# rlorenzo/facet

Measured on AMD Instinct MI355X. Metric: images/sec whole-node (TOPIQ+SAMP+CLIP+InsightFace ensemble), 1024² batch, higher is better.
Workload: dtype f32

## Files before the change

### facet_amd/_lib.py

```python
import ctypes as C
import importlib.util
import os
import sys
import threading

import numpy as np

_HERE = os.path.dirname(os.path.abspath(__file__))
LIB_PATH = os.environ.get("FACET_AMD_LIB") or os.path.join(_HERE, "libfacet_engine.so")

FE_MODEL_TOPIQ, FE_MODEL_CLIP, FE_MODEL_SAMP, FE_MODEL_U2NETP, FE_MODEL_AESTHETIC, FE_MODEL_VLM = range(6)
FE_RECORD_FLOATS = 789
FE_GRAPH_FACE_DET, FE_GRAPH_FACE_LMK, FE_GRAPH_FACE_REC = 0, 1, 2
FE_FACE_FLOATS = 739
FE_STATS_DOUBLES = 264
FILTERS = {"lanczos": 1, "bilinear": 2, "bicubic": 3}
FE_PRECISION_RES32 = 16
FE_PRECISION_SPLIT3 = 32
PRECISION = {"f32": 0, "fp32": 0, "float32": 0, "bf16": 1, "bfloat16": 1, "f16": 2, "fp16": 2, "float16": 2, "half": 2,
             "bf16+r32": 1 | FE_PRECISION_RES32, "f16+r32": 2 | FE_PRECISION_RES32, "f16x3": 2 | FE_PRECISION_RES32 | FE_PRECISION_SPLIT3}
PRECISION_NAME = {0: "f32", 1: "bf16", 2: "f16", 1 | FE_PRECISION_RES32: "bf16+r32", 2 | FE_PRECISION_RES32: "f16+r32",
                  2 | FE_PRECISION_RES32 | FE_PRECISION_SPLIT3: "f16x3"}
ACT = {"none": 0, None: 0, "relu": 1, "gelu": 2, "sigmoid": 3, "softplus": 5, "quickgelu": 6}
ELEM = {"f32": 0, "bf16": 1, "f16": 2}
# ... 31 lines not shown
SIGNATURES = {
    "fe_create": (C.c_int, [C.c_int, C.c_size_t, C.POINTER(C.c_void_p)]),
    "fe_destroy": (None, [C.c_void_p]),
    "fe_last_error": (C.c_char_p, [C.c_void_p]),
    "fe_version": (C.c_char_p, []),
    "fe_sync": (C.c_int, [C.c_void_p]),
    "fe_set_microbatch": (C.c_int, [C.c_void_p, C.c_int]),
    "fe_set_precision": (C.c_int, [C.c_void_p, C.c_int]),
    "fe_model_precision": (C.c_int, [C.c_void_p, C.c_int]),
    "fe_dev_alloc": (C.c_int, [C.c_void_p, C.c_size_t, C.POINTER(C.c_void_p)]),
    "fe_dev_free": (C.c_int, [C.c_void_p, C.c_void_p]),
    "fe_memcpy_h2d": (C.c_int, [C.c_void_p, C.c_void_p, C.c_void_p, C.c_size_t]),
    "fe_memcpy_d2h": (C.c_int, [C.c_void_p, C.c_void_p, C.c_void_p, C.c_size_t]),
    "fe_timer_start": (C.c_int, [C.c_void_p]),
    "fe_timer_stop": (C.c_int, [C.c_void_p, _f32p]),
    "fe_profile_enable": (C.c_int, [C.c_void_p, C.c_int]),
    "fe_profile_count": (C.c_int, [C.c_void_p]),
    "fe_profile_get": (C.c_int, [C.c_void_p, C.c_int, C.c_char_p, C.c_int, C.POINTER(C.c_double),
                                 C.POINTER(C.c_double), _f32p]),
    "fe_flops_reset": (C.c_int, [C.c_void_p]),
    "fe_flops_get": (C.c_int, [C.c_void_p, C.POINTER(C.c_double)]),
    "fe_flops_get_executed": (C.c_int, [C.c_void_p, C.POINTER(C.c_double)]),
    "fe_flops_get_half": (C.c_int, [C.c_void_p, C.POINTER(C.c_double)]),
    "fe_weights_begin": (C.c_int, [C.c_void_p, C.c_int]),
    "fe_weights_set": (C.c_int, [C.c_void_p, C.c_int, C.c_char_p, _f32p, _i64p, C.c_int]),
    "fe_weights_commit": (C.c_int, [C.c_void_p, C.c_int]),
    "fe_model_unload": (C.c_int, [C.c_void_p, C.c_int]),
    "fe_model_loaded": (C.c_int, [C.c_void_p, C.c_int]),
    "fe_op_conv2d": (C.c_int, [C.c_void_p, _f32p, C.c_int, C.c_int, C.c_int, C.c_int, _f32p, C.c_int, C.c_int,
                               C.c_int, _f32p, _f32p, _f32p, C.c_int, C.c_int, C.c_int, C.c_int, C.c_int, _f32p]),
    "fe_op_gate_rowpool": (C.c_int, [C.c_void_p, _f32p, C.c_int, C.c_int, C.c_int, C.c_int, C.c_int, _f32p, _f32p, C.c_int, _f32p, C.c_int,
                                     C.c_int, C.c_int, C.c_int, _f32p, C.POINTER(C.c_int)]),
    "fe_op_wino64": (C.c_int, [C.c_void_p, _f32p, C.c_int, C.c_int, C.c_int, C.c_int, _f32p, C.c_int, _f32p, _f32p, _f32p, C.c_int, C.c_int, _f32p]),
    "fe_op_topiq_gate64": (C.c_int, [C.c_void_p, _f32p, C.c_int, C.c_int, C.c_int, _f32p, _f32p, _f32p, _f32p, _f32p, C.c_float,
                                     _f32p, _f32p, C.c_int, C.c_int, _f32p]),
    "fe_op_conv3x3_c64": (C.c_int, [C.c_void_p, _f32p, C.c_int, C.c_int, C.c_int, _f32p, _f32p, _f32p, C.c_int, _f32p, _f32p, _f32p,
                                    _f32p, _f32p]),
    "fe_op_maxpool2d": (C.c_int, [C.c_void_p, _f32p, C.c_int, C.c_int, C.c_int, C.c_int, C.c_int, C.c_int,
                                  C.c_int, C.c_int, _f32p]),
    "fe_op_bilinear": (C.c_int, [C.c_void_p, _f32p, C.c_int, C.c_int, C.c_int, C.c_int, C.c_int, C.c_int, _f32p]),
    "fe_op_adaptive_avgpool": (C.c_int, [C.c_void_p, _f32p, C.c_int, C.c_int, C.c_int, C.c_int, C.c_int, C.c_int,
                                         _f32p]),
    "fe_op_layernorm": (C.c_int, [C.c_void_p, _f32p, C.c_int, C.c_int, _f32p, _f32p, C.c_float, _f32p]),
    "fe_op_plane": (C.c_int, [C.c_void_p, C.c_int, C.c_int, _f32p] + [C.c_int] * 14 + [C.c_float, C.c_float, _f32p]),
    "fe_op_rowpass": (C.c_int, [C.c_void_p, C.c_int, C.c_int, C.c_int, _f32p] + [C.c_int] * 6 + [_f32p, _f32p, C.c_int, C.c_int, C.c_float, C.c_float, _f32p]),
    "fe_op_gemm_skinny": (C.c_int, [C.c_void_p, C.c_int, C.c_int, C.c_int, _f32p, C.c_int, C.c_int, C.c_int, _f32p, C.c_int, C.c_int, _f32p, _f32p, C.c_int,
                                    C.c_int, C.c_float, _f32p]),
    "fe_op_gemm_skinny_res": (C.c_int, [C.c_void_p, C.c_int, C.c_int, C.c_int, _f32p, C.c_int, C.c_int, C.c_int, _f32p, C.c_int, C.c_int, _f32p, _f32p, _f32p,
                                        C.c_int, C.c_int, C.c_int, C.c_float, _f32p]),
    "fe_op_attention": (C.c_int, [C.c_void_p, _f32p, _f32p, _f32p, _f32p, C.c_int, C.c_int, C.c_int, C.c_int, C.c_int, C.c_int, _f32p]),
    "fe_op_mha": (C.c_int, [C.c_void_p, _f32p, _f32p, C.c_int, C.c_int, C.c_int, C.c_int, C.c_int, _f32p, _f32p, _f32p, _f32p, _f32p,
                            C.c_int, _f32p]),
    "fe_op_vlm_select": (C.c_int, [C.c_void_p, _f32p, C.c_int, C.c_int, C.POINTER(C.c_int32), _f32p]),
    "fe_op_vlm_decode_attention": (C.c_int, [C.c_void_p, _f32p, _f32p, _f32p, C.c_int, C.c_int, C.c_int, C.c_int, C.POINTER(C.c_int32), C.c_int, C.c_int,
                                             _f32p, _f32p, _f32p]),
    "fe_op_vlm_linear": (C.c_int, [C.c_void_p, _f32p, C.c_int, C.c_int, _f32p, _f32p, C.c_int, C.c_int, C.c_int, _f32p, _f32p, _f32p, C.c_float,
                                   C.POINTER(C.c_int32), _f32p, C.c_int, C.c_int, C.c_int, _f32p, _f32p, C.POINTER(C.c_int32)]),
    "fe_op_vlm_rope_cache": (C.c_int, [C.c_void_p, _f32p, C.POINTER(C.c_int32), _f32p, C.c_int, _f32p, _f32p, C.c_float] + [C.c_int] * 12 +
                             [_f32p, C.POINTER(C.c_uint8), C.POINTER(C.c_uint8), _f32p, _f32p]),
    "fe_op_vlm_rows": (C.c_int, [C.c_void_p, C.c_int, _f32p, _f32p, _f32p, C.POINTER(C.c_int32), _f32p, C.c_int, C.c_int, C.c_int, C.c_int, C.c_int,
                                 C.c_float, C.c_int, C.c_int, _f32p, _f32p]),
    "fe_op_vlm_vis_rope": (C.c_int, [C.c_void_p, _f32p, C.POINTER(C.c_int32), _f32p, C.c_int, C.c_int, C.c_int, C.c_int, _f32p, _f32p]),
    "fe_op_vlm_vis_attention": (C.c_int, [C.c_void_p, _f32p, _f32p, _f32p, C.POINTER(C.c_int32), C.c_int, C.c_int, C.c_int, C.c_int, _f32p]),
    "fe_op_vlm_prefill_attention": (C.c_int, [C.c_void_p, _f32p, _f32p, _f32p] + [C.c_int] * 6 + [C.POINTER(C.c_int32), _f32p]),
    "fe_set_conv_variant": (C.c_int, [C.c_void_p, C.c_int]),
    "fe_bench_conv": (C.c_int, [C.c_void_p] + [C.c_int] * 12 + [_f32p]),
# ... 396 lines not shown
        xr, xp = _f32(xr)
        weight, wp = _f32(weight)
        cout = weight.shape[0]
        assert weight.shape == (cout, cin)
        bp = None
        if bias is not None:
            bias, bp = _f32(bias)
        gate, gp = _f32(gate)
        assert gate.shape == (n, h, w)
        y = np.empty((n, th, tw, cout), np.float32)
        routed = C.c_int(0)
        self._ck(self.lib.fe_op_gate_rowpool(self.h, xp, n, h, w, cin, ldx, wp, bp, cout, gp, ACT[act], th, tw, int(bool(fused)),
                                             y.ctypes.data_as(_f32p), C.byref(routed)))
        return np.ascontiguousarray(y.transpose(0, 3, 1, 2)), bool(routed.value)

    def wino64_conv(self, x, w, scale=None, shift=None, res=None, res_after_act=False, act=None):
        x, xp = _f32(x)
        w, wp = _f32(w)
        n, c, h, ww = x.shape
        cout = w.shape[0]
        assert w.shape == (cout, c, 3, 3)
        y = np.empty((n, cout, h, ww), np.float32)
        sp = hp = rp = None
        if scale is not None:
            scale, sp = _f32(scale)
        if shift is not None:
            shift, hp = _f32(shift)
        if res is not None:
            res, rp = _f32(res)
            assert res.shape == y.shape
        self._ck(self.lib.fe_op_wino64(self.h, xp, n, c, h, ww, wp, cout, sp, hp, rp, int(res_after_act), ACT[act], y.ctypes.data_as(_f32p)))
        return y

    def topiq_gate64(self, x, w0, b0, w2, b2, w4, b4, wx, bx, wblk_act="gelu", gate_act="gelu"):
        x, xp = _f32(x)
        n, c, h, w = x.shape
        assert c == 64
        arrs = [_f32(a) for a in (w0, b0, w2, b2, w4, wx, bx)]
        y = np.empty((n, 64, h // 16, w // 16), np.float32)
        self._ck(self.lib.fe_op_topiq_gate64(self.h, xp, n, h, w, arrs[0][1], arrs[1][1], arrs[2][1], arrs[3][1], arrs[4][1], C.c_float(float(b4)),
                                             arrs[5][1], arrs[6][1], ACT[wblk_act], ACT[gate_act], y.ctypes.data_as(_f32p)))
        return y

    def conv3x3_c64(self, x, w2, scale2=None, shift2=None, act2="relu", w3=None, scale3=None, shift3=None, res=None):
        x, xp = _f32(x)
        n, c, h, w = x.shape
        assert c == 64
        keep = [_f32(a) if a is not None else (None, None) for a in (w2, scale2, shift2, w3, scale3, shift3, res)]
        y = np.empty((n, 256 if w3 is not None else 64, h, w), np.float32)
        self._ck(self.lib.fe_op_conv3x3_c64(self.h, xp, n, h, w, keep[0][1], keep[1][1], keep[2][1], ACT[act2], keep[3][1], keep[4][1], keep[5][1],
                                            keep[6][1], y.ctypes.data_as(_f32p)))
        return y

    def maxpool2d(self, x, k, stride, pad=0, ceil_mode=False):
        x, xp = _f32(x)
        n, c, h, w = x.shape

        def od(i):
            if ceil_mode:
                o = -(-(i + 2 * pad - k) // stride) + 1
                if (o - 1) * stride >= i + pad:
                    o -= 1
                return o
            return (i + 2 * pad - k) // stride + 1
        y = np.empty((n, c, od(h), od(w)), np.float32)
        self._ck(self.lib.fe_op_maxpool2d(self.h, xp, n, c, h, w, k, stride, pad, int(ceil_mode),
# ... 1315 lines not shown
```

### facet_amd/csrc/capi_ops.hip

```cpp
#include "capi_internal.h"
#include "fp8_core.h"
#include "wino64_maps.h"

template <class E>
static E* hook_up(Ctx& C, const float* src, size_t n, int off = 0) {
  if (!src) return nullptr;
  if constexpr (std::is_same_v<E, float>) {
    float* d = C.arena.array<float>(n + off) + off;
    FE_HIP(hipMemcpyAsync(d, src, n * sizeof(float), hipMemcpyHostToDevice, C.stream));
    return d;
  } else {
    const float* d32 = upload(C, src, n);
    E* d = C.arena.array<E>(n + off) + off;
    launch_convert(d32, d, n, C.stream);
    return d;
  }
}
template <class E>
static E* hook_filled(Ctx& C, size_t n, float fill, int off = 0) {
  const std::vector<float> v(n, fill);
  E* d = hook_up<E>(C, v.data(), n, off);
  FE_HIP(hipStreamSynchronize(C.stream));
  return d;
}
// ... 123 lines not shown
    FE_HIP(hipMemcpyAsync(xt.p, x, xt.numel() * sizeof(float), hipMemcpyHostToDevice, C.stream));
    Tensor gt = C.arena.tensor(n, h, w, 1);
    FE_HIP(hipMemcpyAsync(gt.p, gate, gt.numel() * sizeof(float), hipMemcpyHostToDevice, C.stream));
    ConvOpts og; og.act = act; og.gate = &gt;
    int took = 0;
    Tensor pooled = topiq_gate_pool(C, cw, xt.slice(0, cw.CinPad), og, th, tw, fused != 0, &took);
    FE_CHECK(pooled.h == th && pooled.w == tw && pooled.ld == cout, "fe_op_gate_rowpool: unexpected result shape");
    FE_HIP(hipMemcpyAsync(y, pooled.p, pooled.numel() * sizeof(float), hipMemcpyDeviceToHost, C.stream));
    FE_HIP(hipStreamSynchronize(C.stream));
    if (routed) *routed = took;
  });
}

int fe_op_wino64(fe_ctx* ctx, const float* x, int n, int c, int h, int w, const float* weight, int cout, const float* scale, const float* shift,
                 const float* res, int res_after_act, int act, float* y) {
  return fe_api(ctx, [&] {
    Ctx& C = ctx->c;
    FE_CHECK(x && weight && y && n > 0 && h > 0 && w > 0 && c > 0 && c <= 64 && c % 4 == 0 && cout > 0 && cout <= 64 && cout % 4 == 0, "bad wino64 arguments");
    FE_CHECK(C.precision == PREC_F32, "fe_op_wino64: fp32 contexts only");
    C.arena.reset();
    std::vector<float> U(w64::U_FLOATS);
    w64::pack_u(weight, cout, c, U.data());
    const float* dU = upload(C, U.data(), U.size());
    const float *ds = upload(C, scale, (size_t)cout), *dh = upload(C, shift, (size_t)cout);
    Tensor xt = upload_nchw(C, x, n, c, h, w, c);
    Tensor rt;
    if (res) rt = upload_nchw(C, res, n, cout, h, w, cout);
    Tensor yt = C.arena.tensor(n, h, w, cout);
    launch_wino64(xt, yt, dU, ds, dh, nullptr, act, res ? &rt : nullptr, res_after_act, C.stream);
    download_nchw(C, yt, cout, y);
  });
}

int fe_op_topiq_gate64(fe_ctx* ctx, const float* x, int n, int h, int w, const float* w0, const float* b0, const float* w2, const float* b2,
                       const float* w4, float b4, const float* wx, const float* bx, int wblk_act, int gate_act, float* y) {
  return fe_api(ctx, [&] {
    Ctx& C = ctx->c;
    FE_CHECK(x && w0 && b0 && w2 && b2 && w4 && wx && bx && y && n > 0 && h > 0 && w > 0 && h % 16 == 0 && w % 16 == 0, "bad gate64 arguments");
    FE_CHECK(C.precision == PREC_BF16 || C.precision == PREC_F16, "fe_op_topiq_gate64: the fused gate exists for the 2-byte element types only");
    C.arena.reset();
    DeviceWeights dw;
    dw.prec = C.precision;
    GatedConvW g;
    build_gate64_fragments(dw, g, w0, b0, w2, b2, w4, b4, wx, bx);
    auto run = [&](auto* tag) {
      typedef std::remove_pointer_t<decltype(tag)> E;
      TensorT<E> xt = upload_nchw<E>(C, x, n, 64, h, w, 64);
      TensorT<E> yt = C.arena.tensor_t<E>(n, h / 16, w / 16, 64);
      launch_topiq_gate64(xt, yt, g.fused, g.fused_bias, wblk_act, gate_act, C.stream);
      download_nchw(C, yt, 64, y);
    };
    if (C.precision == PREC_BF16) run((bf16*)nullptr); else run((f16*)nullptr);
  });
}

int fe_op_conv3x3_c64(fe_ctx* ctx, const float* x, int n, int h, int w, const float* w2, const float* scale2, const float* shift2, int act2,
                      const float* w3, const float* scale3, const float* shift3, const float* res, float* y) {
  return fe_api(ctx, [&] {
    Ctx& C = ctx->c;
    FE_CHECK(x && w2 && y && n > 0 && h > 0 && w > 0 && (!w3 || res), "bad conv3x3_c64 arguments");
    FE_CHECK(C.precision == PREC_BF16 || C.precision == PREC_F16, "fe_op_conv3x3_c64: the halo-tiled kernel exists for the 2-byte element types only");
    C.arena.reset();
    DeviceWeights dw;
    dw.prec = C.precision;
    void *f2 = nullptr, *f3 = nullptr;
    build_c64_fragments(dw, w2, w3, &f2, &f3);
// ... 618 lines not shown
```

### facet_amd/csrc/engine.hip

```cpp
#include "engine.h"
#include "onnx_graph.h"
#include "wino64_maps.h"
#include <algorithm>
#include <cmath>
#include <cstdlib>

namespace fe {

void WeightStore::set(const std::string& name, const float* data, const int64_t* shape, int ndim) {
  HostTensor h;
  h.shape.assign(shape, shape + ndim);
  h.data.assign(data, data + h.numel());
  t_[name] = std::move(h);
}
const HostTensor& WeightStore::get(const std::string& name) const {
  auto it = t_.find(name);
  if (it == t_.end()) throw Error("missing weight tensor '" + name + "'");
  return it->second;
}

float* DeviceWeights::upload(const std::vector<float>& v) {
  void* p = nullptr;
  const size_t b = v.size() * sizeof(float);
  FE_HIP(hipMalloc(&p, b ? b : 16));
// ... 225 lines not shown
}

bool conv_wino64(Ctx& c, const ConvW& w, const Tensor& x, const Tensor& y, const ConvOpts& o) {
  if (!(w.wino64 && c.force_variant == 0 && w.KH == 3 && w.KW == 3 && o.sh == 1 && o.sw == 1 && o.ph == 1 && o.pw == 1 && o.dh == 1 && o.dw == 1 && !o.gate && !o.pool_kw &&
        x.c == w.CinPad && y.c == w.Cout && y.n == x.n && y.h == x.h && y.w == x.w &&
        (((uintptr_t)x.p | (uintptr_t)y.p | (uintptr_t)(o.res ? o.res->p : nullptr)) & 15) == 0 && x.ld % 4 == 0 && y.ld % 4 == 0 &&
        (!o.res || o.res->ld % 4 == 0) && (unsigned long long)x.h * x.w * x.ld * 4ull < 0xF0000000ull && y.pixels() < (1ull << 31)))
    return false;
  const int M = (int)y.pixels();
  hipEvent_t e0 = nullptr, e1 = nullptr;
  if (c.profile) {
    FE_HIP(hipEventCreate(&e0)); FE_HIP(hipEventCreate(&e1));
    FE_HIP(hipEventRecord(e0, c.stream));
  }
  launch_wino64(x, y, w.wino64, w.scale, w.shift, w.slope, o.act, o.res, o.res_after_act, c.stream);
  const double direct = 2.0 * M * (double)(9 * w.Cin) * (w.CoutAlg ? w.CoutAlg : w.Cout);
  if (c.profile) {
    FE_HIP(hipEventRecord(e1, c.stream));
    FE_HIP(hipEventSynchronize(e1));
    float ms = 0.f;
    FE_HIP(hipEventElapsedTime(&ms, e0, e1));
    (void)hipEventDestroy(e0); (void)hipEventDestroy(e1);
    char nm[128];
    snprintf(nm, sizeof nm, "wino64 3x3 M=%d K=%d N=%d", M, w.K, w.Cout);
    const double bytes = 4.0 * ((double)x.pixels() * x.c + (double)y.pixels() * y.c * (o.res ? 2 : 1) + (double)w64::U_FLOATS);
    c.timings.push_back({nm, direct, bytes, ms});
  }
  const double tiles = (double)x.n * ((x.h + 1) / 2) * ((x.w + 1) / 2);
  c.flops_accum += direct;
  c.flops_saved += direct - 2.0 * 16.0 * tiles * 64.0 * w.Cout;
  return true;
}

void conv_forward(Ctx& c, const ConvW& w, const Tensor& x, const Tensor& y, const ConvOpts& o) {
  FE_CHECK(x.c == w.CinPad, "conv: input channels %d != packed Cin %d", x.c, w.CinPad);
  FE_CHECK(y.c == w.Cout && y.n == x.n, "conv: output view mismatch (c=%d Cout=%d)", y.c, w.Cout);
  ConvParams p{};
  p.x = x.p; p.ldx = x.ld;
  p.w = w.w; p.scale = w.scale; p.shift = w.shift; p.slope = w.slope;
  FE_CHECK(o.act != ACT_PRELU || w.slope, "conv: PReLU without slopes");
  if (o.res) {
    FE_CHECK(o.res->c == y.c && o.res->pixels() == y.pixels(), "conv: residual shape mismatch");
    p.res = o.res->p; p.ldr = o.res->ld;
  }
  if (o.gate) {
    FE_CHECK(o.gate->pixels() == y.pixels() && (o.gate->c == 1 || o.gate->c == y.c), "conv: gate shape mismatch");
    p.gate = o.gate->p; p.ldg = o.gate->ld; p.gate_c1 = o.gate->c == 1;
  }
  p.y = y.p; p.ldy = y.ld;
  p.N = x.n; p.H = x.h; p.W = x.w; p.Cin = w.CinPad;
  p.Ho = y.h; p.Wo = y.w; p.Cout = w.Cout;
  p.KH = w.KH; p.KW = w.KW; p.sh = o.sh; p.sw = o.sw; p.ph = o.ph; p.pw = o.pw; p.dh = o.dh; p.dw = o.dw;
  FE_CHECK(y.h == conv_out_dim(x.h, w.KH, o.sh, o.ph, o.dh) && y.w == conv_out_dim(x.w, w.KW, o.sw, o.pw, o.dw),
           "conv: output dims %dx%d inconsistent with input %dx%d", y.h, y.w, x.h, x.w);
  p.K = w.K; p.Kp = w.Kp;
  p.M = (int)y.pixels();
  FE_CHECK(y.pixels() < (1ull << 31), "conv: M too large");
  p.act = o.act; p.res_after_act = o.res_after_act;
  p.variant = c.force_variant;
  if (o.pool_kw) {
    FE_CHECK(conv_rowpool_ok(c, w, x, o, o.pool_kw), "conv: the row-pooling epilogue does not apply to this layer (kw=%d)", o.pool_kw);
    FE_CHECK(o.pool && o.pool->p && o.pool->n == x.n && o.pool->h == x.h && o.pool->w * o.pool_kw == x.w && o.pool->c == w.Cout, "conv: pool view mismatch");
    p.pool_kw = o.pool_kw; p.pool = o.pool->p; p.ldp = o.pool->ld;
    p.y = nullptr; p.ldy = w.Cout;
  }
  if (w.wtap && o.act != ACT_PRELU && o.sh == 1 && o.sw == 1 && !o.res && !o.gate && p.variant == 0 && y.h == x.h && y.w == x.w) {
    const int T = w.KH * w.KW * w.Cout, Tp = (T + 3) & ~3;
    const size_t mark = c.arena.mark();
    Tensor z = c.arena.tensor(x.n, x.h, x.w, Tp);
    ConvParams q{};
    q.x = x.p; q.ldx = x.ld; q.w = w.wtap; q.y = z.p; q.ldy = Tp;
    q.N = x.n; q.H = x.h; q.W = x.w; q.Cin = w.CinPad; q.Ho = x.h; q.Wo = x.w; q.Cout = T;
    q.KH = q.KW = 1; q.sh = q.sw = q.dh = q.dw = 1;
    q.K = w.CinPad; q.Kp = w.KpT; q.M = (int)x.pixels();
    launch_conv(q, c.stream);
    launch_tap_gather(z.p, Tp, x.n, x.h, x.w, w.KH, w.KW, o.ph, o.pw, o.dh, o.dw, w.Cout, w.scale, w.shift, o.act, y.p,
                      y.ld, y.h, y.w, c.stream);
    c.arena.rewind(mark);
    c.flops_accum += 2.0 * p.M * (double)(w.KH * w.KW * w.Cin) * (w.CoutAlg ? w.CoutAlg : p.Cout);
    return;
  }
  static const bool no_wino = getenv("FE_NO_WINO") != nullptr;
  const bool wino_plain = !o.res && (o.act == ACT_NONE || o.act == ACT_RELU);
  if (w.wino && !no_wino && p.variant == 0 && o.sh == 1 && o.sw == 1 && o.ph == 1 && o.pw == 1 && o.dh == 1 && o.dw == 1 &&
      !o.gate && (wino_plain || (w.wino_m == 4 && (o.act == ACT_NONE || o.act == ACT_RELU || o.act == ACT_PRELU))) && y.h == x.h && y.w == x.w && (((uintptr_t)x.p | (uintptr_t)y.p) & 15) == 0 &&
      x.ld % 4 == 0 && y.ld % 4 == 0) {
    const int ts = w.wino_m, planes = (ts + 2) * (ts + 2);
    const int th = (x.h + ts - 1) / ts, tw = (x.w + ts - 1) / ts;
    const size_t tiles = (size_t)x.n * th * tw;
    const size_t wino_bytes = (size_t)planes * tiles * ((size_t)w.CinPad + w.Cout) * sizeof(float) + 1024;
    if (tiles < (1u << 30) / 36 && c.arena.mark() + wino_bytes <= c.arena.capacity()) {
      const size_t mark = c.arena.mark();
      float* V = (float*)c.arena.alloc((size_t)planes * tiles * w.CinPad * sizeof(float));
      float* Mb = (float*)c.arena.alloc((size_t)planes * tiles * w.Cout * sizeof(float));
      hipEvent_t e0 = nullptr, e1 = nullptr;
      if (c.profile) {
        FE_HIP(hipEventCreate(&e0)); FE_HIP(hipEventCreate(&e1));
        FE_HIP(hipEventRecord(e0, c.stream));
      }
      if (ts == 2) launch_wino_input(x, th, tw, V, c.stream);
      else launch_wino4_input(x, th, tw, V, c.stream);
      ConvParams g{};
      g.x = V; g.ldx = w.CinPad; g.w = w.wino; g.ldw = w.CinPad; g.y = Mb; g.ldy = w.Cout;
      g.M = (int)tiles; g.K = w.CinPad; g.Cout = w.Cout;
      g.N = 1; g.H = 1; g.W = g.M; g.Ho = 1; g.Wo = g.M; g.KH = g.KW = 1; g.sh = g.sw = g.dh = g.dw = 1;
      g.Kp = w.CinPad; g.Cin = w.CinPad;
      g.batch = planes; g.nb1 = 1; g.xs2 = (long long)tiles * w.CinPad; g.ws2 = (long long)w.Cout * w.CinPad; g.ys2 = (long long)tiles * w.Cout;
      launch_conv(g, c.stream);
      if (ts == 2) launch_wino_output(Mb, y, th, tw, w.scale, w.shift, o.act == ACT_RELU, c.stream);
      else launch_wino4_output(Mb, y, th, tw, w.scale, w.shift, o.act, w.slope, o.res, o.res_after_act, c.stream);
      if (c.profile) {
        FE_HIP(hipEventRecord(e1, c.stream));
        FE_HIP(hipEventSynchronize(e1));
        float ms = 0.f;
        FE_HIP(hipEventElapsedTime(&ms, e0, e1));
        (void)hipEventDestroy(e0); (void)hipEventDestroy(e1);
        char nm[128];
        snprintf(nm, sizeof nm, "wino3x3 M=%d K=%d N=%d", p.M, p.K, p.Cout);
        c.timings.push_back({nm, 2.0 * p.M * (double)(9 * w.Cin) * p.Cout, 0.0, ms});
      }
      c.arena.rewind(mark);
      c.flops_accum += 2.0 * p.M * (double)(w.KH * w.KW * w.Cin) * (w.CoutAlg ? w.CoutAlg : p.Cout);
      c.flops_saved += 2.0 * p.M * (double)(9 * w.Cin) * (w.CoutAlg ? w.CoutAlg : p.Cout) - 2.0 * (double)planes * (double)tiles * w.CinPad * w.Cout;
      return;
    }
  }
  static const bool no_wino64 = getenv("FE_NO_WINO64") != nullptr;
  if (!no_wino64 && (o.act == ACT_NONE || o.act == ACT_RELU || o.act == ACT_PRELU) && conv_wino64(c, w, x, y, o)) return;
  static const bool no_splitk = getenv("FE_NO_SPLITK") != nullptr;
  static const int splitk_min = getenv("FE_SPLITK_MIN") ? atoi(getenv("FE_SPLITK_MIN")) : 2048;
  if (!no_splitk && w.KH == 1 && w.KW == 1 && o.sh == 1 && o.sw == 1 && o.ph == 0 && o.pw == 0 && !o.gate && p.variant == 0 && p.M <= 256 &&
      w.CinPad >= splitk_min && w.K == w.CinPad && (size_t)((p.M + 127) / 128) * ((w.Cout + 63) / 64) < 64 &&
      (o.act == ACT_NONE || o.act == ACT_RELU || o.act == ACT_PRELU)) {
    int splits = 0;
    for (int s = 64; s >= 2; --s)
      if (w.CinPad % s == 0 && (w.CinPad / s) % 32 == 0 && w.CinPad / s >= 256) { splits = s; break; }
    const size_t part_bytes = (size_t)splits * p.M * w.Cout * sizeof(float);
    if (splits && c.arena.mark() + part_bytes + 1024 <= c.arena.capacity()) {
      const size_t mark = c.arena.mark();
      float* part = (float*)c.arena.alloc(part_bytes);
      const int Ks = w.CinPad / splits;
      hipEvent_t e0 = nullptr, e1 = nullptr;
      if (c.profile) {
        FE_HIP(hipEventCreate(&e0)); FE_HIP(hipEventCreate(&e1));
        FE_HIP(hipEventRecord(e0, c.stream));
      }
      ConvParams g{};
      g.x = x.p; g.ldx = x.ld; g.w = w.w; g.ldw = w.Kp; g.y = part; g.ldy = w.Cout;
      g.M = p.M; g.K = Ks; g.Kp = Ks; g.Cin = Ks; g.Cout = w.Cout;
      g.N = 1; g.H = 1; g.W = g.M; g.Ho = 1; g.Wo = g.M; g.KH = g.KW = 1; g.sh = g.sw = g.dh = g.dw = 1;
      g.batch = splits; g.nb1 = 1; g.xs2 = Ks; g.ws2 = Ks; g.ys2 = (long long)p.M * w.Cout;
      launch_conv(g, c.stream);
      launch_splitk_reduce(part, splits, p.M, w.Cout, w.scale, w.shift, w.slope, o.act, o.res ? o.res->p : nullptr, o.res ? o.res->ld : 0,
                           o.res_after_act, y.p, y.ld, c.stream);
      if (c.profile) {
        FE_HIP(hipEventRecord(e1, c.stream));
        FE_HIP(hipEventSynchronize(e1));
        float ms = 0.f;
        FE_HIP(hipEventElapsedTime(&ms, e0, e1));
        (void)hipEventDestroy(e0); (void)hipEventDestroy(e1);
        char nm[128];
// ... 532 lines not shown
```

### facet_amd/csrc/fe_common.h

```cpp
#pragma once
#include <hip/hip_runtime.h>
#include "fe_check.h"
#include "erf_core.h"
#include "stats_plan.h"
#include "face_mixed_plan.h"
#include "composition_mixed_plan.h"
#include <cstdint>
#include <cstdio>
#include <atomic>
#include <cstring>
#include <map>
#include <mutex>
#include <stdexcept>
#include <string>
#include <utility>
#include <vector>

namespace fe {


#define FE_HIP(expr)                                                                      \
  do {                                                                                    \
    hipError_t _e = (expr);                                                               \
    if (_e != hipSuccess) {                                                               \
// ... 237 lines not shown
  int hprec = 0;
  int KpH = 0, cb = 0, CinPadH = 0;
  void* wtap_h = nullptr;
  int KpTH = 0;
  uint8_t* w8 = nullptr;
  float* w8_scale = nullptr;
};

template <class T>
struct ConvOptsT {
  int sh = 1, sw = 1, ph = 0, pw = 0, dh = 1, dw = 1;
  int act = ACT_NONE;
  const TensorT<T>* res = nullptr;
  int res_after_act = 0;
  const TensorT<T>* gate = nullptr;
  const TensorT<float>* res32 = nullptr;
  const TensorT<float>* y32 = nullptr;
  int pool_kw = 0;
  const TensorT<T>* pool = nullptr;
};
using ConvOpts = ConvOptsT<float>;

constexpr int CONV_KALIGN = 32;
constexpr int CONV_KALIGN_H = 64;

void launch_conv(const ConvParams& p, hipStream_t s);
void launch_wino_input(const Tensor& x, int th, int tw, float* V, hipStream_t s);
void launch_wino_output(const float* Mb, const Tensor& y, int th, int tw, const float* scale, const float* shift, int relu, hipStream_t s);
void launch_wino4_input(const Tensor& x, int th, int tw, float* V, hipStream_t s);
void launch_wino4_output(const float* Mb, const Tensor& y, int th, int tw, const float* scale, const float* shift, int act, const float* slope,
                         const Tensor* res, int res_after_act, hipStream_t s);
void launch_wino64(const Tensor& x, const Tensor& y, const float* U, const float* scale, const float* shift, const float* slope, int act,
                   const Tensor* res, int res_after_act, hipStream_t s);
template <class TO>
bool launch_stem(const float* x, int ldx, int N, int H, int W, const float* wstem, const float* scale, const float* shift, const float* slope,
                 int Cout, int k, int stride, int act, TO* y, int ldy, int Ho, int Wo, hipStream_t s);
void launch_conv_narrow(const ConvParams& p, hipStream_t s);
void launch_conv_dma(const ConvParams& p, int tile, hipStream_t s);
void launch_conv_bf16(const ConvParamsH& p, hipStream_t s);
void launch_conv_bf16(const ConvParamsT<f16>& p, hipStream_t s);
template <class T, class Launch>
inline bool conv_split_by_images(const ConvParamsT<T>& p, Launch&& launch) {
  if (p.batch > 1 || p.N <= 1 || (long long)p.N * p.Ho * p.Wo != (long long)p.M) return false;
  const unsigned long long in_img = (unsigned long long)p.H * p.W * p.ldx * sizeof(T);
  unsigned long long out_img = (unsigned long long)p.Ho * p.Wo * (unsigned long long)(p.ldy > p.ldr ? p.ldy : p.ldr) * sizeof(T);
  const unsigned long long out32_img = (unsigned long long)p.Ho * p.Wo * (unsigned long long)(p.ldy32 > p.ldr32 ? p.ldy32 : p.ldr32) * sizeof(float);
  if ((p.y32 || p.res32) && out32_img > out_img) out_img = out32_img;
  const unsigned long long per_img = in_img > out_img ? in_img : out_img;
  constexpr unsigned long long LIMIT = 0xF0000000ull;
  if (per_img >= LIMIT) return false;
  const int ng = (int)(LIMIT / per_img);
  if (ng >= p.N) return false;
  for (int i0 = 0; i0 < p.N; i0 += ng) {
    ConvParamsT<T> q = p;
    const int n = ng < p.N - i0 ? ng : p.N - i0;
    const size_t opix = (size_t)i0 * p.Ho * p.Wo;
    q.N = n; q.M = n * p.Ho * p.Wo;
    q.x = p.x + (size_t)i0 * p.H * p.W * p.ldx;
    if (p.y) q.y = p.y + opix * p.ldy;
    if (p.y32) q.y32 = p.y32 + opix * p.ldy32;
    if (p.res32) q.res32 = p.res32 + opix * p.ldr32;
    if (p.res) q.res = p.res + opix * p.ldr;
    if (p.gate) q.gate = p.gate + opix * p.ldg;
    if (p.pool_kw) q.pool = p.pool + opix / p.pool_kw * p.ldp;
    launch(q);
  }
// ... 114 lines not shown
```

### include/facet_engine.h

```cpp
#ifndef FACET_ENGINE_H
#define FACET_ENGINE_H

#include <stddef.h>
#include <stdint.h>

#ifdef __cplusplus
extern "C" {
#endif

typedef struct fe_ctx fe_ctx;

enum fe_status {
  FE_OK = 0,
  FE_ERR_INVALID = -1,
  FE_ERR_RUNTIME = -2,
  FE_ERR_NOT_LOADED = -3,
  FE_ERR_CAPACITY = -4
};

enum fe_model {
  FE_MODEL_TOPIQ = 0,
  FE_MODEL_CLIP = 1,
  FE_MODEL_SAMP = 2,
  FE_MODEL_U2NETP = 3,
// ... 53 lines not shown
                          int32_t* out_tokens, float* out_logprobs, int* steps_run);

int fe_dev_alloc(fe_ctx* ctx, size_t bytes, void** d_out);
int fe_dev_free(fe_ctx* ctx, void* d_ptr);
int fe_memcpy_h2d(fe_ctx* ctx, void* d_dst, const void* src, size_t bytes);
int fe_memcpy_d2h(fe_ctx* ctx, void* dst, const void* d_src, size_t bytes);

int fe_timer_start(fe_ctx* ctx);
int fe_timer_stop(fe_ctx* ctx, float* ms_out);
int fe_profile_enable(fe_ctx* ctx, int on);
int fe_profile_count(fe_ctx* ctx);
int fe_profile_get(fe_ctx* ctx, int i, char* name, int name_cap, double* flops, double* bytes, float* ms);
int fe_flops_reset(fe_ctx* ctx);
int fe_flops_get(fe_ctx* ctx, double* flops);
int fe_flops_get_executed(fe_ctx* ctx, double* flops);
int fe_flops_get_half(fe_ctx* ctx, double* flops);

int fe_weights_begin(fe_ctx* ctx, int model);
int fe_weights_set(fe_ctx* ctx, int model, const char* name, const float* data, const int64_t* shape, int ndim);
int fe_weights_commit(fe_ctx* ctx, int model);
int fe_model_unload(fe_ctx* ctx, int model);
int fe_model_loaded(fe_ctx* ctx, int model);

int fe_op_conv2d(fe_ctx* ctx, const float* x, int n, int c, int h, int w, const float* weight, int cout, int kh,
                 int kw, const float* scale, const float* shift, const float* res, int res_after_act, int stride,
                 int pad, int dil, int act, float* y);
int fe_op_topiq_gate64(fe_ctx* ctx, const float* x, int n, int h, int w, const float* w0, const float* b0, const float* w2,
                       const float* b2, const float* w4, float b4, const float* wx, const float* bx, int wblk_act,
                       int gate_act, float* y);
int fe_op_gate_rowpool(fe_ctx* ctx, const float* x, int n, int h, int w, int cin, int ldx, const float* weight, const float* bias, int cout,
                       const float* gate, int act, int th, int tw, int fused, float* y, int* routed);
int fe_op_wino64(fe_ctx* ctx, const float* x, int n, int c, int h, int w, const float* weight, int cout, const float* scale, const float* shift,
                 const float* res, int res_after_act, int act, float* y);
int fe_op_conv3x3_c64(fe_ctx* ctx, const float* x, int n, int h, int w, const float* w2, const float* scale2,
                      const float* shift2, int act2, const float* w3, const float* scale3, const float* shift3,
                      const float* res, float* y);
int fe_op_maxpool2d(fe_ctx* ctx, const float* x, int n, int c, int h, int w, int k, int stride, int pad,
                    int ceil_mode, float* y);
int fe_op_bilinear(fe_ctx* ctx, const float* x, int n, int c, int h, int w, int ho, int wo, float* y);
int fe_op_adaptive_avgpool(fe_ctx* ctx, const float* x, int n, int c, int h, int w, int ho, int wo, float* y);
int fe_op_layernorm(fe_ctx* ctx, const float* x, int rows, int d, const float* g, const float* b, float eps, float* y);
#define FE_ELEM_F32 0
#define FE_ELEM_BF16 1
#define FE_ELEM_F16 2
int fe_op_plane(fe_ctx* ctx, int route, int elem, const float* x, int n, int c, int h, int w, int ctot_in, int c0_in, int ctot_out, int c0_out,
                int k, int stride, int pad, int ceil_mode, int ho, int wo, float poison, float fill, float* y);
int fe_op_rowpass(fe_ctx* ctx, int route, int elem_in, int elem_out, const float* x, int rows, int d, int ldx, int ldy, int off_x, int off_y,
                  const float* g, const float* b, int off_gb, int L, float eps, float fill, float* y);
int fe_op_gemm_skinny(fe_ctx* ctx, int ti, int tw, int to, const float* x, int M, int K, int ldx, const float* w, int N, int ldw,
                      const float* scale, const float* shift, int act, int ldy, float fill, float* y);
int fe_op_gemm_skinny_res(fe_ctx* ctx, int ti, int tw, int to, const float* x, int M, int K, int ldx, const float* w, int N, int ldw,
                          const float* scale, const float* shift, const float* res, int ldr, int act, int ldy, float fill, float* y);
int fe_op_attention(fe_ctx* ctx, const float* q, const float* k, const float* v, const float* bv, int B, int H, int Lq, int Lk,
                    int causal, int form, float* o);
int fe_op_mha(fe_ctx* ctx, const float* x_q, const float* x_kv, int B, int Lq, int Lk, int d, int heads, const float* in_proj_weight,
              const float* in_proj_bias, const float* out_proj_weight, const float* out_proj_bias, const float* res, int causal,
              float* y);
int fe_op_vlm_select(fe_ctx* ctx, const float* logits, int rows, int vocab, int32_t* ids, float* logprobs);
int fe_op_vlm_decode_attention(fe_ctx* ctx, const float* q, const float* k, const float* v, int B, int nh, int nkv, int Lk, const int32_t* pad, int kv_format,
                               int len_from_device, float* out, float* k_image, float* v_image);
int fe_op_vlm_linear(fe_ctx* ctx, const float* x, int M, int ldx, const float* w, const float* bias, int N, int K, int weight_format, const float* w2,
                     const float* xres, const float* g, float eps, const int32_t* slot, const float* ds, int n_ds, int route, int kernel, float* y,
                     float* y2, int32_t* info);
int fe_op_vlm_rope_cache(fe_ctx* ctx, const float* qkv, const int32_t* pos, const float* inv_freq, int family, const float* qn, const float* kn, float eps,
                         int sa, int sb, int B, int L, int nh, int nkv, int start, int start_from_device, int max_seq, int kv_format, int max_blocks, int fill,
                         float* q_out, uint8_t* k_raw, uint8_t* v_raw, float* k_scale, float* v_scale);
// ... 221 lines not shown
```

Baseline: 244.2.

## Add persistent MFMA streaming kernel for large fp32 1x1 convolutions

Adds a persistent kernel for 1x1 convolutions that keeps the whole weight matrix in LDS and streams row blocks of pixels, prefetching the next block's activations in registers. It uses fp32 MFMA with a fused scale/shift, activation and residual epilogue written through per-wave LDS strips. Routing covers large 64->256 and 64->64 convolutions and the 64-channel tap GEMM of the tap-gather path. It targets the memory-bound 1x1 layers that the generic conv kernel handles less efficiently; the cost is more code paths and an extra pass through LDS in the epilogue.

Result: no change. 246.6, median of 6 (+1.0%).

```diff
diff --git a/facet_amd/_lib.py b/facet_amd/_lib.py
--- a/facet_amd/_lib.py
+++ b/facet_amd/_lib.py
@@ -87,6 +87,8 @@
     "fe_op_gate_rowpool": (C.c_int, [C.c_void_p, _f32p, C.c_int, C.c_int, C.c_int, C.c_int, C.c_int, _f32p, _f32p, C.c_int, _f32p, C.c_int,
                                      C.c_int, C.c_int, C.c_int, _f32p, C.POINTER(C.c_int)]),
     "fe_op_wino64": (C.c_int, [C.c_void_p, _f32p, C.c_int, C.c_int, C.c_int, C.c_int, _f32p, C.c_int, _f32p, _f32p, _f32p, C.c_int, C.c_int, _f32p]),
+    "fe_op_stream1x1": (C.c_int, [C.c_void_p, _f32p, C.c_int, C.c_int, C.c_int, _f32p, C.c_int, C.c_int, _f32p, _f32p, _f32p, C.c_int, C.c_int,
+                                  C.c_int, C.c_int, C.c_int, C.c_float, _f32p]),
     "fe_op_topiq_gate64": (C.c_int, [C.c_void_p, _f32p, C.c_int, C.c_int, C.c_int, _f32p, _f32p, _f32p, _f32p, _f32p, C.c_float,
                                      _f32p, _f32p, C.c_int, C.c_int, _f32p]),
     "fe_op_conv3x3_c64": (C.c_int, [C.c_void_p, _f32p, C.c_int, C.c_int, C.c_int, _f32p, _f32p, _f32p, C.c_int, _f32p, _f32p, _f32p,
@@ -549,6 +551,32 @@
         self._ck(self.lib.fe_op_wino64(self.h, xp, n, c, h, ww, wp, cout, sp, hp, rp, int(res_after_act), ACT[act], y.ctypes.data_as(_f32p)))
         return y
 
+    def stream1x1_conv(self, x, w, scale=None, shift=None, res=None, res_after_act=False, act=None, cout=None, ldy=None, store_cols=None,
+                       fill=3e4):
+        x, xp = _f32(x)
+        w, wp = _f32(w)
+        m, ldx = x.shape
+        wrows, cin = w.shape
+        cout = wrows if cout is None else int(cout)
+        store_cols = cout if store_cols is None else int(store_cols)
+        ldy = store_cols if ldy is None else int(ldy)
+        sp = hp = rp = None
+        ldr = 0
+        if scale is not None:
+            scale, sp = _f32(scale)
+            assert scale.shape == (cout,)
+        if shift is not None:
+            shift, hp = _f32(shift)
+            assert shift.shape == (cout,)
+        if res is not None:
+            res, rp = _f32(res)
+            assert res.shape[0] == m
+            ldr = res.shape[1]
+        y = np.empty((m, ldy), np.float32)
+        self._ck(self.lib.fe_op_stream1x1(self.h, xp, m, cin, ldx, wp, wrows, cout, sp, hp, rp, ldr, int(res_after_act), ACT[act], ldy, store_cols,
+                                          C.c_float(float(fill)), y.ctypes.data_as(_f32p)))
+        return y
+
     def topiq_gate64(self, x, w0, b0, w2, b2, w4, b4, wx, bx, wblk_act="gelu", gate_act="gelu"):
         x, xp = _f32(x)
         n, c, h, w = x.shape
diff --git a/facet_amd/csrc/capi_ops.hip b/facet_amd/csrc/capi_ops.hip
--- a/facet_amd/csrc/capi_ops.hip
+++ b/facet_amd/csrc/capi_ops.hip
@@ -179,6 +179,24 @@
   });
 }
 
+int fe_op_stream1x1(fe_ctx* ctx, const float* x, int m, int cin, int ldx, const float* weight, int wrows, int cout, const float* scale,
+                    const float* shift, const float* res, int ldr, int res_after_act, int act, int ldy, int store_cols, float fill, float* y) {
+  return fe_api(ctx, [&] {
+    Ctx& C = ctx->c;
+    FE_CHECK(x && weight && y && m > 0 && cin > 0 && ldx >= cin && wrows > 0 && cout >= wrows && store_cols > 0 && ldy >= store_cols && (!res || ldr >= cout),
+             "bad stream1x1 arguments");
+    FE_CHECK(C.precision == PREC_F32, "fe_op_stream1x1: fp32 contexts only");
+    C.arena.reset();
+    const float* dx = hook_up<float>(C, x, (size_t)m * ldx);
+    const float* dwt = hook_up<float>(C, weight, (size_t)wrows * cin);
+    const float *ds = hook_up<float>(C, scale, (size_t)cout), *dh = hook_up<float>(C, shift, (size_t)cout);
+    const float* dr = hook_up<float>(C, res, (size_t)m * ldr);
+    float* dy = hook_filled<float>(C, (size_t)m * ldy, fill);
+    launch_stream1x1(dx, ldx, cin, dy, ldy, cout, store_cols, m, dwt, cin, wrows, ds, dh, act, dr, ldr, res_after_act, C.stream);
+    hook_down(C, dy, (size_t)m * ldy, y);
+  });
+}
+
 int fe_op_topiq_gate64(fe_ctx* ctx, const float* x, int n, int h, int w, const float* w0, const float* b0, const float* w2, const float* b2,
                        const float* w4, float b4, const float* wx, const float* bx, int wblk_act, int gate_act, float* y) {
   return fe_api(ctx, [&] {
diff --git a/facet_amd/csrc/engine.hip b/facet_amd/csrc/engine.hip
--- a/facet_amd/csrc/engine.hip
+++ b/facet_amd/csrc/engine.hip
@@ -281,6 +281,48 @@
   return true;
 }
 
+static bool stream1x1_routed_shape(int Cin, int Cout) {
+  return (Cin == 64 && Cout == 256) || (Cin == 64 && Cout == 64);
+}
+constexpr size_t STREAM1X1_MIN_BYTES = (size_t)2 << 20, STREAM1X1_TAP_MIN_BYTES = (size_t)1 << 20;
+static bool stream1x1_large(const Tensor& x, int Cout, size_t min_bytes) {
+  return (size_t)x.h * x.w * (size_t)(x.c > Cout ? x.c : Cout) * sizeof(float) >= min_bytes;
+}
+
+static bool conv_stream1x1(Ctx& c, const ConvW& w, const Tensor& x, const Tensor& y, const ConvOpts& o) {
+  if (!(w.KH == 1 && w.KW == 1 && o.sh == 1 && o.sw == 1 && o.ph == 0 && o.pw == 0 && o.dh == 1 && o.dw == 1 && !o.gate && !o.pool_kw && c.force_variant == 0 &&
+        (o.act == ACT_NONE || o.act == ACT_RELU || o.act == ACT_GELU) && w.w && x.c == w.CinPad && w.Kp == w.CinPad && y.c == w.Cout && y.n == x.n && y.h == x.h &&
+        y.w == x.w && stream1x1_shape_ok(w.CinPad, w.Cout) && stream1x1_routed_shape(w.CinPad, w.Cout) && stream1x1_large(x, w.Cout, STREAM1X1_MIN_BYTES)))
+    return false;
+  auto al16 = [](const void* ptr) { return ((uintptr_t)ptr & 15) == 0; };
+  if (!(al16(x.p) && al16(y.p) && al16(w.w) && al16(w.scale) && al16(w.shift) && x.ld % 4 == 0 && y.ld % 4 == 0 && (!o.res || (al16(o.res->p) && o.res->ld % 4 == 0)) &&
+        y.pixels() < (1ull << 31) - 65536))
+    return false;
+  if (getenv("FE_NO_STREAM1X1")) return false;
+  const int M = (int)y.pixels();
+  hipEvent_t e0 = nullptr, e1 = nullptr;
+  if (c.profile) {
+    FE_HIP(hipEventCreate(&e0)); FE_HIP(hipEventCreate(&e1));
+    FE_HIP(hipEventRecord(e0, c.stream));
+  }
+  launch_stream1x1(x.p, x.ld, w.CinPad, y.p, y.ld, w.Cout, w.Cout, M, w.w, w.Kp, w.Cout, w.scale, w.shift, o.act, o.res ? o.res->p : nullptr, o.res ? o.res->ld : 0,
+                   o.res_after_act, c.stream);
+  const double flops = 2.0 * M * (double)w.Cin * (w.CoutAlg ? w.CoutAlg : w.Cout);
+  if (c.profile) {
+    FE_HIP(hipEventRecord(e1, c.stream));
+    FE_HIP(hipEventSynchronize(e1));
+    float ms = 0.f;
+    FE_HIP(hipEventElapsedTime(&ms, e0, e1));
+    (void)hipEventDestroy(e0); (void)hipEventDestroy(e1);
+    char nm[128];
+    snprintf(nm, sizeof nm, "stream1x1 M=%d K=%d N=%d", M, w.K, w.Cout);
+    const double bytes = 4.0 * ((double)x.pixels() * x.c + (double)y.pixels() * y.c * (o.res ? 2 : 1) + (double)w.Cout * w.K);
+    c.timings.push_back({nm, flops, bytes, ms});
+  }
+  c.flops_accum += flops;
+  return true;
+}
+
 void conv_forward(Ctx& c, const ConvW& w, const Tensor& x, const Tensor& y, const ConvOpts& o) {
   FE_CHECK(x.c == w.CinPad, "conv: input channels %d != packed Cin %d", x.c, w.CinPad);
   FE_CHECK(y.c == w.Cout && y.n == x.n, "conv: output view mismatch (c=%d Cout=%d)", y.c, w.Cout);
@@ -322,7 +364,25 @@
     q.N = x.n; q.H = x.h; q.W = x.w; q.Cin = w.CinPad; q.Ho = x.h; q.Wo = x.w; q.Cout = T;
     q.KH = q.KW = 1; q.sh = q.sw = q.dh = q.dw = 1;
     q.K = w.CinPad; q.Kp = w.KpT; q.M = (int)x.pixels();
-    launch_conv(q, c.stream);
+    hipEvent_t e0 = nullptr, e1 = nullptr;
+    if (c.profile) {
+      FE_HIP(hipEventCreate(&e0)); FE_HIP(hipEventCreate(&e1));
+      FE_HIP(hipEventRecord(e0, c.stream));
+    }
+    const bool s1 = !getenv("FE_NO_STREAM1X1") && T <= 32 && w.CinPad == 64 && w.KpT == w.CinPad && stream1x1_large(x, 32, STREAM1X1_TAP_MIN_BYTES) &&
+                    ((uintptr_t)x.p & 15) == 0 && x.ld % 4 == 0 && x.pixels() < (1ull << 31) - 65536;
+    if (s1) launch_stream1x1(x.p, x.ld, w.CinPad, z.p, Tp, 32, Tp, q.M, w.wtap, w.KpT, T, nullptr, nullptr, ACT_NONE, nullptr, 0, 0, c.stream);
+    else launch_conv(q, c.stream);
+    if (c.profile) {
+      FE_HIP(hipEventRecord(e1, c.stream));
+      FE_HIP(hipEventSynchronize(e1));
+      float ms = 0.f;
+      FE_HIP(hipEventElapsedTime(&ms, e0, e1));
+      (void)hipEventDestroy(e0); (void)hipEventDestroy(e1);
+      char nm[128];
+      snprintf(nm, sizeof nm, "%s M=%d K=%d N=%d", s1 ? "stream1x1 wtap" : "conv1x1 wtap", q.M, w.CinPad, T);
+      c.timings.push_back({nm, 2.0 * q.M * (double)w.CinPad * T, 4.0 * ((double)x.pixels() * x.c + (double)x.pixels() * Tp + (double)T * w.CinPad), ms});
+    }
     launch_tap_gather(z.p, Tp, x.n, x.h, x.w, w.KH, w.KW, o.ph, o.pw, o.dh, o.dw, w.Cout, w.scale, w.shift, o.act, y.p,
                       y.ld, y.h, y.w, c.stream);
     c.arena.rewind(mark);
@@ -376,6 +436,7 @@
   }
   static const bool no_wino64 = getenv("FE_NO_WINO64") != nullptr;
   if (!no_wino64 && (o.act == ACT_NONE || o.act == ACT_RELU || o.act == ACT_PRELU) && conv_wino64(c, w, x, y, o)) return;
+  if (conv_stream1x1(c, w, x, y, o)) return;
   static const bool no_splitk = getenv("FE_NO_SPLITK") != nullptr;
   static const int splitk_min = getenv("FE_SPLITK_MIN") ? atoi(getenv("FE_SPLITK_MIN")) : 2048;
   if (!no_splitk && w.KH == 1 && w.KW == 1 && o.sh == 1 && o.sw == 1 && o.ph == 0 && o.pw == 0 && !o.gate && p.variant == 0 && p.M <= 256 &&
diff --git a/facet_amd/csrc/fe_common.h b/facet_amd/csrc/fe_common.h
--- a/facet_amd/csrc/fe_common.h
+++ b/facet_amd/csrc/fe_common.h
@@ -293,6 +293,9 @@
                          const Tensor* res, int res_after_act, hipStream_t s);
 void launch_wino64(const Tensor& x, const Tensor& y, const float* U, const float* scale, const float* shift, const float* slope, int act,
                    const Tensor* res, int res_after_act, hipStream_t s);
+bool stream1x1_shape_ok(int Cin, int Cout);
+void launch_stream1x1(const float* x, int ldx, int Cin, float* y, int ldy, int Cout, int store_cols, long long M, const float* w, int ldw, int wrows,
+                      const float* scale, const float* shift, int act, const float* res, int ldr, int res_after_act, hipStream_t s);
 template <class TO>
 bool launch_stem(const float* x, int ldx, int N, int H, int W, const float* wstem, const float* scale, const float* shift, const float* slope,
                  int Cout, int k, int stride, int act, TO* y, int ldy, int Ho, int Wo, hipStream_t s);
diff --git a/facet_amd/csrc/kernels_stream1x1.hip b/facet_amd/csrc/kernels_stream1x1.hip
--- /dev/null
+++ b/facet_amd/csrc/kernels_stream1x1.hip
@@ -0,0 +1,175 @@
+#include "fe_common.h"
+#include "stream1x1_maps.h"
+
+namespace fe {
+
+struct S1Params {
+  const float* x; int ldx;
+  float* y; int ldy;
+  const float* w; int ldw, wrows;
+  const float *scale, *shift;
+  const float* res; int ldr;
+  int res_after_act, act;
+  int M, nblocks;
+  int store_cols;
+};
+
+template <int A>
+struct S1Act { static constexpr int value = A; };
+
+template <int KS, int NJ>
+__global__ __launch_bounds__(256, 1) void stream1x1_kernel(const S1Params p) {
+  using namespace s1;
+  constexpr int NQ = 2 * KS;
+  constexpr int NCH = (NJ + 1) / 2;
+  constexpr int NF = KS * 16 * NJ * 32 / 4;
+  extern __shared__ __attribute__((aligned(16))) float smem[];
+  const int t = threadIdx.x, lane = t & 63, wave = __builtin_amdgcn_readfirstlane(t >> 6);
+  const int r = lane & 31, h = lane >> 5;
+
+  fe_v4f* const sW = reinterpret_cast<fe_v4f*>(smem);
+  for (int f = t; f < NF; f += 256) {
+    const int row = b_src_row(f, NJ), col = b_src_col(f, NJ);
+    fe_v4f v = {0.f, 0.f, 0.f, 0.f};
+    if (row < p.wrows) v = *reinterpret_cast<const fe_v4f*>(p.w + (size_t)row * p.ldw + col);
+    sW[f] = v;
+  }
+  __syncthreads();
+  float* const E = smem + NF * 4 + wave * STRIP_FLOATS;
+  const fe_v4f* const bw = sW + lane;
+
+  float4 sc[NCH], sf[NCH];
+#pragma unroll
+  for (int cc = 0; cc < NCH; ++cc) {
+    const int cw = chunk_width(cc, NJ);
+    const int col = cc * CHUNK + epi_col(lane, cw);
+    sc[cc] = p.scale ? *reinterpret_cast<const float4*>(p.scale + col) : make_float4(1.f, 1.f, 1.f, 1.f);
+    sf[cc] = p.shift ? *reinterpret_cast<const float4*>(p.shift + col) : make_float4(0.f, 0.f, 0.f, 0.f);
+  }
+
+  fe_v4f a[NQ], an[NQ];
+  auto fetch_a = [&](const int v, fe_v4f (&dst)[NQ]) __attribute__((always_inline)) {
+    const int m = clamp_row(wave_row0(clamp_block(v, p.nblocks), wave) + r, p.M);
+    const float* const src = p.x + (size_t)m * p.ldx + 4 * h;
+#pragma unroll
+    for (int q = 0; q < NQ; ++q) dst[q] = *reinterpret_cast<const fe_v4f*>(src + 8 * q);
+  };
+  constexpr int NRES = NCH * 8;
+  float4 rv[NRES];
+
+  fetch_a(blockIdx.x, a);
+  for (int v = blockIdx.x; v < p.nblocks; v += gridDim.x) {
+    const int row0 = wave_row0(v, wave);
+    if (p.res) {
+#pragma unroll
+      for (int cc = 0; cc < NCH; ++cc) {
+        const int cw = chunk_width(cc, NJ);
+#pragma unroll
+        for (int it = 0; it < epi_iters(cw); ++it) {
+          const int m = clamp_row(row0 + epi_row(lane, it, cw), p.M);
+          rv[cc * 8 + it] = *reinterpret_cast<const float4*>(p.res + (size_t)m * p.ldr + cc * CHUNK + epi_col(lane, cw));
+        }
+      }
+    }
+    fetch_a(v + (int)gridDim.x, an);
+    __builtin_amdgcn_sched_barrier(0);
+
+    fe_f32x16 acc[NJ];
+#pragma unroll
+    for (int j = 0; j < NJ; ++j)
+#pragma unroll
+      for (int e = 0; e < 16; ++e) acc[j][e] = 0.f;
+#pragma unroll
+    for (int q = 0; q < NQ; ++q) {
+      fe_v4f fb[NJ];
+#pragma unroll
+      for (int j = 0; j < NJ; ++j) fb[j] = bw[b_frag(q, j, 0, NJ)];
+#pragma unroll
+      for (int c = 0; c < 4; ++c)
+#pragma unroll
+        for (int j = 0; j < NJ; ++j) acc[j] = __builtin_amdgcn_mfma_f32_32x32x2f32(a[q][c], fb[j][c], acc[j], 0, 0, 0);
+    }
+
+#pragma unroll
+    for (int cc = 0; cc < NCH; ++cc) {
+      const int cw = chunk_width(cc, NJ);
+      const int nj = cw / 32;
+#pragma unroll
+      for (int jj = 0; jj < 2; ++jj)
+        if (jj < nj) {
+#pragma unroll
+          for (int e = 0; e < 16; ++e) E[strip_index(acc_row(e, h), jj * 32 + r)] = acc[2 * cc + jj][e];
+        }
+      const int lc = epi_col(lane, cw), colb = cc * CHUNK + lc;
+      const bool cok = colb < p.store_cols;
+      const float4 s4 = sc[cc], f4 = sf[cc];
+      auto finish = [&](auto actc) __attribute__((always_inline)) {
+        constexpr int act = decltype(actc)::value;
+#pragma unroll
+        for (int it = 0; it < epi_iters(cw); ++it) {
+          const int er = epi_row(lane, it, cw), m = row0 + er;
+          float4 u = *reinterpret_cast<const float4*>(&E[strip_index(er, lc)]);
+          const float4 rr = rv[cc * 8 + it];
+          u.x = u.x * s4.x + f4.x; u.y = u.y * s4.y + f4.y; u.z = u.z * s4.z + f4.z; u.w = u.w * s4.w + f4.w;
+          if (p.res && !p.res_after_act) { u.x += rr.x; u.y += rr.y; u.z += rr.z; u.w += rr.w; }
+          u.x = fe_apply_act(u.x, act); u.y = fe_apply_act(u.y, act); u.z = fe_apply_act(u.z, act); u.w = fe_apply_act(u.w, act);
+          if (p.res && p.res_after_act) { u.x += rr.x; u.y += rr.y; u.z += rr.z; u.w += rr.w; }
+          if (cok && m < p.M) *reinterpret_cast<float4*>(p.y + (size_t)m * p.ldy + colb) = u;
+        }
+      };
+      if (p.act == ACT_RELU) finish(S1Act<ACT_RELU>{});
+      else if (p.act == ACT_GELU) finish(S1Act<ACT_GELU>{});
+      else finish(S1Act<ACT_NONE>{});
+    }
+#pragma unroll
+    for (int q = 0; q < NQ; ++q) a[q] = an[q];
+  }
+}
+
+template <int KS, int NJ>
+static void launch_s1_variant(const S1Params& p, hipStream_t s) {
+  constexpr size_t lds = ((size_t)KS * 16 * NJ * 32 + (size_t)s1::WAVES * s1::STRIP_FLOATS) * sizeof(float);
+  static_assert(lds < 160 * 1024, "weights + strips must fit LDS");
+  auto kern = stream1x1_kernel<KS, NJ>;
+  static std::atomic<uint64_t> lds_set{0};
+  ensure_dynamic_lds((const void*)kern, lds, lds_set);
+  static const int per_cu = [&] {
+    int n = 1;
+    if (hipOccupancyMaxActiveBlocksPerMultiprocessor(&n, (const void*)kern, 256, lds) != hipSuccess) { (void)hipGetLastError(); n = 1; }
+    return n < 1 ? 1 : (n > 3 ? 3 : n);
+  }();
+  const int slots = 256 * per_cu;
+  const int grid = p.nblocks < slots ? p.nblocks : slots;
+  hipLaunchKernelGGL(kern, dim3(grid), dim3(256), lds, s, p);
+  FE_HIP(hipGetLastError());
+}
+
+bool stream1x1_shape_ok(int Cin, int Cout) {
+  return Cin > 0 && Cout > 0 && Cin % 32 == 0 && Cout % 32 == 0 && Cin <= s1::MAX_C && Cout <= s1::MAX_C && Cin * Cout <= s1::MAX_W_FLOATS;
+}
+
+void launch_stream1x1(const float* x, int ldx, int Cin, float* y, int ldy, int Cout, int store_cols, long long M, const float* w, int ldw, int wrows,
+                      const float* scale, const float* shift, int act, const float* res, int ldr, int res_after_act, hipStream_t s) {
+  auto al16 = [](const void* ptr) { return ((uintptr_t)ptr & 15) == 0; };
+  FE_CHECK(stream1x1_shape_ok(Cin, Cout), "stream1x1: %d -> %d channels (multiples of 32, <= 256, Cin * Cout <= 16384)", Cin, Cout);
+  FE_CHECK(x && y && w && M > 0 && M < (1ll << 31) - 65536, "stream1x1: null operand or bad row count %lld", M);
+  FE_CHECK(ldx % 4 == 0 && ldy % 4 == 0 && ldw % 4 == 0 && ldx >= Cin && ldw >= Cin && (!res || ldr % 4 == 0), "stream1x1: leading dimensions must be multiples of 4");
+  FE_CHECK(al16(x) && al16(y) && al16(w) && al16(scale) && al16(shift) && al16(res), "stream1x1: operands must be 16-byte aligned");
+  FE_CHECK(store_cols > 0 && store_cols % 4 == 0 && store_cols <= Cout && ldy >= store_cols && (!res || ldr >= Cout), "stream1x1: bad output / residual view");
+  FE_CHECK(wrows > 0 && wrows <= Cout, "stream1x1: %d weight rows for %d columns", wrows, Cout);
+  FE_CHECK(act == ACT_NONE || act == ACT_RELU || act == ACT_GELU, "stream1x1: activation %d", act);
+  S1Params p{};
+  p.x = x; p.ldx = ldx; p.y = y; p.ldy = ldy; p.w = w; p.ldw = ldw; p.wrows = wrows;
+  p.scale = scale; p.shift = shift; p.res = res; p.ldr = ldr; p.res_after_act = res_after_act; p.act = act;
+  p.M = (int)M; p.nblocks = s1::row_blocks((int)M); p.store_cols = store_cols;
+  const int k2 = Cin / 32, nj = Cout / 32;
+#define S1_CASE(K2, NJ) if (k2 == K2 && nj == NJ) { launch_s1_variant<2 * K2, NJ>(p, s); return; }
+#define S1_ROW(K2, N1) S1_CASE(K2, 1) if constexpr (N1 >= 2) S1_CASE(K2, 2) if constexpr (N1 >= 3) S1_CASE(K2, 3) if constexpr (N1 >= 4) S1_CASE(K2, 4) \
+  if constexpr (N1 >= 5) S1_CASE(K2, 5) if constexpr (N1 >= 6) S1_CASE(K2, 6) if constexpr (N1 >= 7) S1_CASE(K2, 7) if constexpr (N1 >= 8) S1_CASE(K2, 8)
+  S1_ROW(1, 8) S1_ROW(2, 8) S1_ROW(3, 5) S1_ROW(4, 4) S1_ROW(5, 3) S1_ROW(6, 2) S1_ROW(7, 2) S1_ROW(8, 2)
+#undef S1_ROW
+#undef S1_CASE
+  FE_CHECK(false, "stream1x1: no kernel for %d -> %d", Cin, Cout);
+}
+
+}
diff --git a/facet_amd/csrc/stream1x1_maps.h b/facet_amd/csrc/stream1x1_maps.h
--- /dev/null
+++ b/facet_amd/csrc/stream1x1_maps.h
@@ -0,0 +1,51 @@
+#pragma once
+
+#if defined(__HIPCC__)
+#define S1_HD __host__ __device__ __forceinline__
+#else
+#define S1_HD inline
+#endif
+
+namespace fe {
+namespace s1 {
+
+constexpr int WAVES = 4;
+constexpr int WAVE_ROWS = 32;
+constexpr int BLOCK_ROWS = WAVES * WAVE_ROWS;
+constexpr int SLAB = 16;
+constexpr int CHUNK = 64;
+constexpr int ES = CHUNK + 4;
+constexpr int STRIP_FLOATS = WAVE_ROWS * ES;
+constexpr int MAX_C = 256;
+constexpr int MAX_W_FLOATS = 16384;
+
+S1_HD int row_blocks(int M) { return (M + BLOCK_ROWS - 1) / BLOCK_ROWS; }
+S1_HD int wave_row0(int v, int wave) { return v * BLOCK_ROWS + wave * WAVE_ROWS; }
+S1_HD int clamp_row(int m, int M) { return m < M ? m : M - 1; }
+S1_HD int clamp_block(int v, int nblocks) { return v < nblocks ? v : nblocks - 1; }
+
+S1_HD int a_col(int q, int h) { return 8 * q + 4 * h; }
+S1_HD int a_k(int s, int hh, int c, int h) { return a_col(2 * s + hh, h) + c; }
+S1_HD int dma_k(int s, int hh, int c, int r, int h) {
+  const int sw = (r >> 2) & 3;
+  const int fo0 = (h ^ sw) << 2, fo1 = fo0 ^ 8;
+  const int slot = (hh ? fo1 : fo0) >> 2;
+  return SLAB * s + 4 * (slot ^ sw) + c;
+}
+
+S1_HD int b_frag(int q, int j, int lane, int NJ) { return (q * NJ + j) * 64 + lane; }
+S1_HD int b_frag_count(int Cin, int Cout) { return Cin * Cout / 4; }
+S1_HD int b_src_row(int f, int NJ) { return ((f >> 6) % NJ) * 32 + (f & 31); }
+S1_HD int b_src_col(int f, int NJ) { return 8 * ((f >> 6) / NJ) + 4 * ((f >> 5) & 1); }
+
+S1_HD int acc_row(int e, int h) { return (e & 3) + 8 * (e >> 2) + 4 * h; }
+S1_HD int strip_index(int row, int col) { return row * ES + col; }
+S1_HD int epi_lanes_per_row(int cw) { return cw / 4; }
+S1_HD int epi_iters(int cw) { return WAVE_ROWS / (64 / epi_lanes_per_row(cw)); }
+S1_HD int epi_row(int lane, int it, int cw) { return lane / epi_lanes_per_row(cw) + it * (64 / epi_lanes_per_row(cw)); }
+S1_HD int epi_col(int lane, int cw) { return (lane % epi_lanes_per_row(cw)) * 4; }
+S1_HD int chunks(int NJ) { return (NJ + 1) / 2; }
+S1_HD int chunk_width(int cc, int NJ) { return 2 * cc + 1 < NJ ? CHUNK : 32; }
+
+}
+}
diff --git a/include/facet_engine.h b/include/facet_engine.h
--- a/include/facet_engine.h
+++ b/include/facet_engine.h
@@ -109,6 +109,8 @@
                        const float* gate, int act, int th, int tw, int fused, float* y, int* routed);
 int fe_op_wino64(fe_ctx* ctx, const float* x, int n, int c, int h, int w, const float* weight, int cout, const float* scale, const float* shift,
                  const float* res, int res_after_act, int act, float* y);
+int fe_op_stream1x1(fe_ctx* ctx, const float* x, int m, int cin, int ldx, const float* weight, int wrows, int cout, const float* scale,
+                    const float* shift, const float* res, int ldr, int res_after_act, int act, int ldy, int store_cols, float fill, float* y);
 int fe_op_conv3x3_c64(fe_ctx* ctx, const float* x, int n, int h, int w, const float* w2, const float* scale2,
                       const float* shift2, int act2, const float* w3, const float* scale3, const float* shift3,
                       const float* res, float* y);
```
